# Kelicious/faster_rcnn

Measured on AMD Instinct MI355X. Metric: images/sec end-to-end (RPN+det) ResNet-50 600x1000, higher is better.
Workload: dtype f32

## Files before the change

faster_rcnn_amd/_lib.py:

```python
import ctypes
import os
from ctypes import c_char_p, c_double, c_int, c_size_t, c_void_p

HERE = os.path.dirname(os.path.abspath(__file__))
LIB_PATH = os.environ.get("FRCNN_LIB_PATH") or os.path.join(HERE, "libfrcnn_hip.so")


class FrcnnError(RuntimeError):
    pass


ABI_VERSION = 110
P = c_void_p
I = c_int
SIGNATURES = {
    "frcnn_last_error": (c_char_p, []),
    "frcnn_version": (I, []),
    "frcnn_device_count": (I, []),
    "frcnn_preprocess_u8": (I, [P, c_size_t, P, P, P]),
    "frcnn_resize_cubic_taps": (I, [I, I, P]),
    "frcnn_resize_cubic_u8": (I, [P, I, I, P, P, I, I, I, P, P]),
    "frcnn_anchors_image": (I, [I, I, P, I, I, P, P]),
    "frcnn_anchors_conv": (I, [I, I, P, I, P, P]),
    "frcnn_cross_ious_f32": (I, [P, I, P, I, P, P]),
# ... 109 lines not shown
    "frcnn_annotate_u8": (I, [P, I, I, P, P, P, P, I, P, P, I, I, P, P]),
    "frcnn_vgg_conv1_bf16_packed_elems": (I, []),
    "frcnn_pack_vgg_conv1_weights_bf16": (I, [P, P, P]),
    "frcnn_vgg_conv1_bf16_fwd": (I, [P, I, I, I, P, P, P, P]),
    "frcnn_pool2d_fwd_bf16": (I, [P, I, I, I, I, I, I, P, P]),
}

VGG_CANVAS_VERSION = 1
EXT_SIGNATURES = {
    "frcnn_vgg_canvas_version": (I, []),
    "frcnn_pool2d_fwd_extents": (I, [P, I, I, I, I, P, P, P]),
    "frcnn_pool2d_fwd_bf16_extents": (I, [P, I, I, I, I, P, P, P]),
    "frcnn_vgg_conv1_bf16_fwd_extents": (I, [P, I, I, I, P, P, P, P, P]),
}

ROI_RES_VERSION = 1
ROI_TAP_BYTES = 32
ROI_RES_SIGNATURES = {
    "frcnn_roi_res_version": (I, []),
    "frcnn_roi_tap_table": (I, [I, I, I, P, I, I, I, I, I, P, P]),
    "frcnn_conv2d_roi_res_available": (I, [P, I, I]),
    "frcnn_conv2d_fwd_h3_roi_res": (I, [P, P, P, P, P, P, P, P, P, P, P, P, ctypes.c_float, ctypes.c_float, P]),
}


POOL_EPILOGUE_VERSION = 1
POOL_EPILOGUE_SIGNATURES = {
    "frcnn_pool_epilogue_version": (I, []),
    "frcnn_conv2d_pool_available": (I, [P, I, I, I]),
    "frcnn_conv2d_fwd_h3_pool": (I, [P, P, P, P, P, P, P, P, P, P, I, P, P, P, P]),
}


class RoiRes(ctypes.Structure):
    _fields_ = [("map", c_void_p), ("taps", c_void_p), ("fill", c_void_p), ("map_rows", ctypes.c_int32), ("reserved", ctypes.c_int32)]


PNG_VERSION = 1
PNG_SIGNATURES = {
    "frcnn_png_version": (I, []),
    "frcnn_png_band_rows": (I, []),
    "frcnn_png_bound": (c_size_t, [I, I]),
    "frcnn_png_workspace_bytes": (c_size_t, [I, I]),
    "frcnn_png_encode_u8": (I, [P, I, I, I, P, c_size_t, P, P, P]),
}

PNG_HUFF_VERSION = 1
PNG_HUFF_SIGNATURES = {
    "frcnn_png_huff_version": (I, []),
    "frcnn_png_huff_band_rows": (I, []),
    "frcnn_png_huff_bound": (c_size_t, [I, I]),
    "frcnn_png_huff_workspace_bytes": (c_size_t, [I, I]),
    "frcnn_png_huff_encode_u8": (I, [P, I, I, I, P, c_size_t, P, P, P]),
}

JPEG_VERSION = 1
JPEG_SIGNATURES = {
    "frcnn_jpeg_version": (I, []),
    "frcnn_jpeg_restart_mcus": (I, []),
    "frcnn_jpeg_header_bytes": (c_size_t, []),
    "frcnn_jpeg_bound": (c_size_t, [I, I]),
    "frcnn_jpeg_workspace_bytes": (c_size_t, [I, I]),
    "frcnn_jpeg_encode_u8": (I, [P, I, I, I, I, P, c_size_t, P, P, P]),
}

JPEG_OPT_VERSION = 1
# ... 281 lines not shown
class ColsumJob(ctypes.Structure):
    _fields_ = [(k, c_void_p) for k in ("g", "scale", "out")] + [(k, ctypes.c_int32) for k in ("m", "cout", "g_is_bf16", "reserved")]


_lib = None


def load():
    global _lib
    if _lib is not None:
        return _lib
    if not os.path.exists(LIB_PATH):
        raise FrcnnError(
            f"{LIB_PATH} is missing: build it with `python -m faster_rcnn_amd.build` "
            "(hipcc --offload-arch=gfx950).  There is no CPU fallback.")
    import torch
    lib = ctypes.CDLL(LIB_PATH)
    for name, (res, args) in SIGNATURES.items():
        fn = getattr(lib, name)
        fn.restype = res
        fn.argtypes = args
    for name, (res, args) in EXT_SIGNATURES.items():
        fn = getattr(lib, name)
        fn.restype = res
        fn.argtypes = args
    for name, (res, args) in ROI_RES_SIGNATURES.items():
        fn = getattr(lib, name)
        fn.restype = res
        fn.argtypes = args
    for name, (res, args) in POOL_EPILOGUE_SIGNATURES.items():
        fn = getattr(lib, name)
        fn.restype = res
        fn.argtypes = args
    for name, (res, args) in PNG_SIGNATURES.items():
        fn = getattr(lib, name)
        fn.restype = res
        fn.argtypes = args
    for name, (res, args) in PNG_HUFF_SIGNATURES.items():
        fn = getattr(lib, name)
        fn.restype = res
        fn.argtypes = args
    for name, (res, args) in JPEG_SIGNATURES.items():
        fn = getattr(lib, name)
        fn.restype = res
        fn.argtypes = args
    for name, (res, args) in JPEG_OPT_SIGNATURES.items():
        fn = getattr(lib, name)
        fn.restype = res
        fn.argtypes = args
    for name, (res, args) in JPEG_DEC_SIGNATURES.items():
        fn = getattr(lib, name)
        fn.restype = res
        fn.argtypes = args
    for name, (res, args) in JPEG_DEC_BATCH_SIGNATURES.items():
        fn = getattr(lib, name)
        fn.restype = res
        fn.argtypes = args
    for name, (res, args) in PNG_DEC_SIGNATURES.items():
        fn = getattr(lib, name)
        fn.restype = res
        fn.argtypes = args
    for name, (res, args) in PNG_DEC_FULL_SIGNATURES.items():
        fn = getattr(lib, name)
        fn.restype = res
        fn.argtypes = args
    for name, (res, args) in JPEG_DEC_FULL_SIGNATURES.items():
# ... 144 lines not shown
```

faster_rcnn_amd/csrc/conv_igemm.hip:

```cpp
#include "conv_f32_common.h"
#include "conv_policy.h"
#include "../../include/ext/frcnn_hip_roi_res.h"
#include "../../include/ext/frcnn_hip_pool_epilogue.h"

namespace frcnn {

template <int TM, int TN, bool GENERIC_A>
__global__ void __launch_bounds__(256) k_conv_igemm_f32(const ConvArgs p) {
    constexpr int BM = 64 * TM, BN = 64 * TN;
    constexpr int PA = BM / 32, PB = BN / 32;
    extern __shared__ __attribute__((aligned(16))) float smem[];
    float* As = smem;
    float* Bs = smem + 2 * BM * LDS_STRIDE;

    const int tid = threadIdx.x, lane = tid & 63, wave = tid >> 6;
    const int wm = wave >> 1, wn = wave & 1;
    const int li = lane & 31, lh = lane >> 5;

    const int nwg = p.tiles_m * p.tiles_n;
    const int logical = xcd_remap(blockIdx.x, nwg);
    const int tile_n = logical / p.tiles_m, tile_m = logical - tile_n * p.tiles_m;
    const int m0 = tile_m * BM, n0 = tile_n * BN;

    const int lrow = tid >> 3, lcol = (tid & 7) * 4;
    int a_h[PA], a_w[PA];
    size_t a_img[PA];
#pragma unroll
    for (int i = 0; i < PA; ++i) {
        const int m = m0 + lrow + 32 * i;
        if (m < p.M) {
            const int wo = m % p.Wo, t = m / p.Wo, ho = t % p.Ho, img = t / p.Ho;
            a_h[i] = ho * p.stride - p.pad_top;
            a_w[i] = wo * p.stride - p.pad_left;
            a_img[i] = (size_t)img * p.H * p.W * p.Cin;
        } else {
            a_h[i] = -(1 << 28); a_w[i] = 0; a_img[i] = 0;
// ... 856 lines not shown
    a.img_stride = a.layout ? d->cin : d->h * d->w * d->cin;
    a.inv_S = (65536 + d->kw - 1) / d->kw;
    auto al16 = [](const void* q) { return (reinterpret_cast<uintptr_t>(q) & 15) == 0; };
    a.vec_epi = !conv_knobs().scalar_epilogue && (d->cout & 3) == 0 && (a.ldy & 3) == 0 && al16(y) && (size_t)M * a.ldy * 4 < 0x7fffffffull
             && (!residual || ((a.ldres & 3) == 0 && al16(residual) && (size_t)M * a.ldres * 4 < 0x7fffffffull))
             && (!mask || (al16(mask) && (size_t)M * d->cout * 4 < 0x7fffffffull)) && (!scale || al16(scale)) && (!shift || al16(shift));
    auto dual_vec_epi = [&](int bn) {
        return a.vec_epi && dual->n1 % bn == 0 && (a.ldy2 & 3) == 0 && al16(dual->y2) && (size_t)M * a.ldy2 * 4 < 0x7fffffffull;
    };
    auto use_workspace = [&]() { a.tickets = (unsigned*)workspace; a.slabs = (float*)((char*)workspace + SPLITK_TICKET_BYTES); };
    hipStream_t s = as_stream(stream);
    const bool generic = (d->cin % BK) != 0;
    if (engine != FRCNN_ENGINE_NATIVE) {
        const bool h3 = engine == FRCNN_ENGINE_H3;
        const SplitRule& r = split_rule(engine);
        int (*launch)(const ConvArgs&, int, hipStream_t) = h3 ? launch_conv_h3 : launch_conv_x6;
        if (generic || d->kh * d->kw > 32) return fail(FRCNN_E_UNSUPPORTED, "conv2d_fwd_%s: cin %% 32 == 0 and at most 32 taps", r.name);
        if ((size_t)r.planes * d->cout * a.Kpad * 2 >= 0x7fffffffull) return fail(FRCNN_E_UNSUPPORTED, "conv2d_fwd_%s: filter planes over 2 GiB", r.name);
        if (h3 && (reinterpret_cast<uintptr_t>(w_packed) & 15)) return fail(FRCNN_E_ARG, "conv2d_fwd_h3: 16-byte aligned filter planes required");
        const int cfg = split_config(r, d, dual ? dual->n1 : 0), bn = r.tile_width(cfg);
        if (a.res_map) {
            if (roi_res_available(d, engine, a.x_planes != nullptr) != 1 || dual || mask || residual || a.res_planes || workspace)
                return fail(FRCNN_E_UNSUPPORTED, "conv2d_fwd_h3_roi_res: not available for this launch (frcnn_conv2d_roi_res_available)");
            if (y && !a.vec_epi) return fail(FRCNN_E_ARG, "conv2d_fwd_h3_roi_res: 16-byte addressable output rows required");
            if ((long long)a.res_map_rows * d->cout * 4 >= 0x7fffffffLL || M * 32 >= 0x7fffffffLL) return fail(FRCNN_E_UNSUPPORTED, "conv2d_fwd_h3_roi_res: map or tap table over 2 GiB");
        }
        if (a.pool_rows) {
            if (pool_available(d, engine, a.x_planes != nullptr, a.pool_rows) != 1 || dual || mask || a.res_planes || a.res_map || a.y_planes || workspace || !y)
                return fail(FRCNN_E_UNSUPPORTED, "conv2d_fwd_h3_pool: not available for this launch (frcnn_conv2d_pool_available)");
            if (!a.vec_epi) return fail(FRCNN_E_ARG, "conv2d_fwd_h3_pool: 16-byte addressable output and residual rows required");
            a.pool_groups = 256 / a.pool_rows < 1024 / 128 ? 256 / a.pool_rows : 1024 / 128;
        }
        if (planes_io) {
            if ((cfg != 86 && cfg != 85 && cfg != 82) || dual || mask || (!a.vec_epi && y) || d->ldy > 0)
                return fail(FRCNN_E_UNSUPPORTED, "conv2d_fwd_h3_planes: needs the 256x128 tile (>= 256 output tiles of 128x128; frcnn_conv2d_h3_config 86 / 82), a dense single-layer launch without a mask");
            if ((d->cout & 3) || (d->cin & 7)) return fail(FRCNN_E_UNSUPPORTED, "conv2d_fwd_h3_planes: cin %% 8 == 0 and cout %% 4 == 0");
            if (a.res_planes && (residual || (y && !a.vec_epi))) return fail(FRCNN_E_ARG, "conv2d_fwd_h3_planes: residual planes exclude an f32 residual and need 16-byte addressable output rows");
            if ((size_t)M * d->cout * 4 >= 0x7fffffffull || (size_t)d->n * d->h * d->w * d->cin * 4 >= 0x7fffffffull)
                return fail(FRCNN_E_UNSUPPORTED, "conv2d_fwd_h3_planes: tensor planes over 2 GiB");
            if (!y) a.vec_epi = 1;
        } else if (workspace && !dual) {
            if (const size_t need = split_workspace_bytes(r, d)) {
                if (workspace_bytes < need) return fail(FRCNN_E_WORKSPACE, "conv2d_fwd_%s: workspace needs %zu bytes", r.name, need);
                a.splits = split_slices(r, d);
                use_workspace();
                a.group_m = 0;
                return launch(a, split_sk_code(r, d), s);
            }
        }
        if (dual) a.vec_epi = dual_vec_epi(bn);
        a.group_m = split_group_m(d, bn);
        return launch(a, cfg, s);
    }
    int cfg = choose_config(d);
    if (dual) {
        cfg = dual_config(cfg);
        a.vec_epi = dual_vec_epi(native_tile_width(cfg));
    }
    a.group_m = native_group_m(d, cfg);
    cfg = workspace_config(d, cfg, workspace != nullptr);
    if (a.layout && (generic || cfg < 11 || d->kh * d->kw > 32))
        return fail(FRCNN_E_UNSUPPORTED, "conv2d_fwd: position-major layout needs cin %% 32 == 0, a tensor under 2 GiB and at most 32 taps");
    if (d->cin == 3) {
        if (a.layout) return fail(FRCNN_E_UNSUPPORTED, "conv2d_fwd: position-major layout needs cin %% 32 == 0");
        if ((size_t)d->n * d->h * d->w * 12 >= 0x7fffffffull) return fail(FRCNN_E_UNSUPPORTED, "conv2d_fwd: 3-channel input over 2 GiB");
        return launch_conv_cin3(a, s, d->tile % 100 != 32);
    }
// ... 134 lines not shown

int frcnn_conv2d_fwd_x6(const frcnn_conv_desc* d, const float* x, const void* w_planes_bf16,
                        const float* scale, const float* shift, const float* residual, const float* mask, float* y,
                        void* workspace, size_t workspace_bytes, void* stream) {
    return conv_fwd_impl(d, x, reinterpret_cast<const float*>(w_planes_bf16), scale, shift, residual, mask, y, nullptr, workspace, workspace_bytes, stream, FRCNN_ENGINE_X6);
}

int frcnn_conv2d_fwd_dual_x6(const frcnn_conv_desc* d, const float* x, const void* w_planes_bf16, const float* scale, const float* shift,
                             float* y1, int n1, int act1, float* y2, int act2, void* stream) {
    if (!d || !y2 || n1 <= 0 || n1 >= d->cout) return fail(FRCNN_E_ARG, "conv2d_fwd_dual_x6: need 0 < n1 < cout and two outputs");
    if (d->ldy > 0 || d->ldres > 0) return fail(FRCNN_E_ARG, "conv2d_fwd_dual_x6: dense outputs only (ldy = ldres = 0)");
    const DualOut dual = {n1, act1, y2, act2};
    return conv_fwd_impl(d, x, reinterpret_cast<const float*>(w_planes_bf16), scale, shift, nullptr, nullptr, y1, &dual, nullptr, 0, stream, FRCNN_ENGINE_X6);
}

int frcnn_conv2d_fwd_h3(const frcnn_conv_desc* d, const float* x, const float* x_amax, const void* w_planes_f16,
                        const float* scale, const float* shift, const float* residual, const float* mask, float* y, float* y_amax,
                        void* workspace, size_t workspace_bytes, void* stream) {
    if (!x_amax) return fail(FRCNN_E_ARG, "conv2d_fwd_h3: the input's magnitude record is required (frcnn_amax_f32 makes one)");
    return conv_fwd_impl(d, x, reinterpret_cast<const float*>(w_planes_f16), scale, shift, residual, mask, y, nullptr, workspace, workspace_bytes, stream, FRCNN_ENGINE_H3,
                         amax_args(x_amax, y_amax));
}

int frcnn_conv2d_fwd_dual_h3(const frcnn_conv_desc* d, const float* x, const float* x_amax, const void* w_planes_f16, const float* scale, const float* shift,
                             float* y1, int n1, int act1, float* y1_amax, float* y2, int act2, float* y2_amax, void* stream) {
    if (!d || !y2 || n1 <= 0 || n1 >= d->cout) return fail(FRCNN_E_ARG, "conv2d_fwd_dual_h3: need 0 < n1 < cout and two outputs");
    if (d->ldy > 0 || d->ldres > 0) return fail(FRCNN_E_ARG, "conv2d_fwd_dual_h3: dense outputs only (ldy = ldres = 0)");
    if (!x_amax) return fail(FRCNN_E_ARG, "conv2d_fwd_dual_h3: the input's magnitude record is required");
    const DualOut dual = {n1, act1, y2, act2};
    return conv_fwd_impl(d, x, reinterpret_cast<const float*>(w_planes_f16), scale, shift, nullptr, nullptr, y1, &dual, nullptr, 0, stream, FRCNN_ENGINE_H3,
                         amax_args(x_amax, y1_amax, y2_amax));
}

int frcnn_conv2d_fwd_h3_planes(const frcnn_conv_desc* d, const float* x, const frcnn_h3_planes* x_planes, const float* x_amax, const void* w_planes_f16,
                               const float* scale, const float* shift, const float* residual, const float* residual_amax,
                               float* y, float* y_amax, const frcnn_h3_planes* y_planes, float bound_c, float bound_d, void* stream) {
    return frcnn_conv2d_fwd_h3_planes_res(d, x, x_planes, x_amax, w_planes_f16, scale, shift, residual, nullptr, residual_amax, y, y_amax, y_planes, bound_c, bound_d, stream);
}

int frcnn_conv2d_roi_res_available(const frcnn_conv_desc* d, int engine, int x_is_planes) {
    if (!d) return fail(FRCNN_E_ARG, "conv2d_roi_res_available: null descriptor");
    if (engine != FRCNN_ENGINE_NATIVE && engine != FRCNN_ENGINE_X6 && engine != FRCNN_ENGINE_H3) return fail(FRCNN_E_ARG, "conv2d_roi_res_available: unknown engine %d", engine);
    return roi_res_available(d, engine, x_is_planes != 0);
}

int frcnn_conv2d_fwd_h3_roi_res(const frcnn_conv_desc* d, const float* x, const frcnn_h3_planes* x_planes, const float* x_amax,
                                const void* w_planes_f16, const float* scale, const float* shift, const frcnn_roi_res* res,
                                const float* residual_amax, float* y, float* y_amax, const frcnn_h3_planes* y_planes,
                                float bound_c, float bound_d, void* stream) {
    return conv_h3_planes_impl(d, x, x_planes, x_amax, w_planes_f16, scale, shift, nullptr, nullptr, res, residual_amax, y, y_amax, y_planes, bound_c, bound_d, stream);
}

int frcnn_conv2d_fwd_h3_planes_res(const frcnn_conv_desc* d, const float* x, const frcnn_h3_planes* x_planes, const float* x_amax, const void* w_planes_f16,
                                   const float* scale, const float* shift, const float* residual, const frcnn_h3_planes* residual_planes,
                                   const float* residual_amax, float* y, float* y_amax, const frcnn_h3_planes* y_planes, float bound_c, float bound_d,
                                   void* stream) {
    return conv_h3_planes_impl(d, x, x_planes, x_amax, w_planes_f16, scale, shift, residual, residual_planes, nullptr, residual_amax, y, y_amax, y_planes, bound_c, bound_d, stream);
}

}

static int conv_h3_planes_impl(const frcnn_conv_desc* d, const float* x, const frcnn_h3_planes* x_planes, const float* x_amax, const void* w_planes_f16,
                               const float* scale, const float* shift, const float* residual, const frcnn_h3_planes* residual_planes,
                               const frcnn_roi_res* gathered, const float* residual_amax, float* y, float* y_amax, const frcnn_h3_planes* y_planes,
                               float bound_c, float bound_d, void* stream) {
    if (gathered) {
// ... 24 lines not shown
```

faster_rcnn_amd/nets.py:

```python
import os as _os

import numpy as np
import torch

from . import ops
from .weights import VGG_CONVS, resnet_block_names

BN_EPS_STEM = 1e-3
BN_EPS_BLOCK = 1e-5


class ConvUnit:

    def __init__(self, weights, conv, bn=None, scale=None, eps=BN_EPS_BLOCK, stride=1, padding="valid", act=None, tile=0,
                 dtype="f32", out_f32=False):
        self.weights, self.conv, self.bn, self.scale_name, self.eps = weights, conv, bn, scale, eps
        self.stride, self.padding, self.act, self.tile = stride, padding, act, tile
        self.dtype, self.out_f32 = dtype, out_f32
        self.pc = None

    def folded(self):
        w = self.weights[self.conv]
        kernel = np.asarray(w[0], dtype=np.float32)
        if kernel.ndim == 2:
# ... 33 lines not shown
        h, w = (x.shape[0], x.shape[1]) if layout else (x.shape[1], x.shape[2])
        return ops.conv2d_avgpool(x, self.pc, self.stride, self.padding, self.act, residual, h * w, self.tile, layout)


class DualUnit:

    def __init__(self, first, second):
        assert first.dtype == second.dtype == "f32" and (first.stride, first.padding) == (second.stride, second.padding)
        self.a, self.b, self.pc, self.n1 = first, second, None, None
        self._src = None

    def lower(self):
        a, b = self.a, self.b
        for u in (a, b):
            if u.pc is None:
                u.lower()
        wa, wb = a.pc.w, b.pc.w
        pc = ops.PackedConv.__new__(ops.PackedConv)
        pc.kh, pc.kw, pc.cin, pc.cout = a.pc.kh, a.pc.kw, a.pc.cin, a.pc.cout + b.pc.cout
        assert (a.pc.kh, a.pc.kw, a.pc.cin) == (b.pc.kh, b.pc.kw, b.pc.cin)
        pc.w = torch.cat([wa, wb], dim=0).contiguous()
        pc.scale = torch.cat([a.pc.scale, b.pc.scale]).contiguous()
        pc.shift = torch.cat([a.pc.shift, b.pc.shift]).contiguous()
        self.pc, self.n1, self._src = pc, a.pc.cout, (a.pc, b.pc)
        return self

    def __call__(self, x, act1="unit", act2="unit", layout=0):
        if self.pc is None or self._src[0] is not self.a.pc or self._src[1] is not self.b.pc:
            self.lower()
        act1 = self.a.act if act1 == "unit" else act1
        act2 = self.b.act if act2 == "unit" else act2
        return ops.conv2d_dual(x, self.pc, self.n1, self.a.stride, self.a.padding, act1, act2, layout, self.a.tile)


FUSE_PAIRS = True
FUSED_BF16_STEM = True
FUSED_F32_STEM = True


def _pair(first, second):
    if not FUSE_PAIRS or first.dtype != "f32" or second.dtype != "f32":
        return None
    d = getattr(first, "_dual", None)
    if d is None or d.b is not second:
        w = first.weights[first.conv][0]
        if np.ndim(w) != 4 or np.shape(w)[2] % 32 != 0:
            return None
        d = first._dual = DualUnit(first, second)
    return d


def _block_units(weights, stage, block, has_shortcut, stride, separate_scale, dtype="f32"):
    def unit(suffix, **kw):
        tag = "%d%s_branch%s" % (stage, block, suffix)
        return ConvUnit(weights, "res" + tag, "bn" + tag, ("scale" + tag) if separate_scale else None, BN_EPS_BLOCK, dtype=dtype, **kw)
    u = {"2a": unit("2a", stride=stride, act="relu"),
         "2b": unit("2b", padding="same", act="relu"),
         "2c": unit("2c", act="relu")}
    if has_shortcut:
        u["1"] = unit("1", stride=stride)
    return u


HEAD_PLANES = True
HEAD_BLOCK_PLANES = _os.environ.get("FRCNN_HEAD_BLOCK_PLANES", "0") != "0"
HEAD_ROI_RES = _os.environ.get("FRCNN_HEAD_ROI_RES", "1") != "0"
HEAD_POOL_EPI = _os.environ.get("FRCNN_HEAD_POOL_EPI", "1") != "0"
VGG_PLANES = _os.environ.get("FRCNN_VGG_PLANES", "1") != "0"
TRUNK_PLANES = _os.environ.get("FRCNN_TRUNK_PLANES", "0") != "0"


class Extents:
    LEVELS = 3
    CONV_LEVEL = 2

    @staticmethod
    def offset_of(height, width):
        return height & 1, width & 1

    def __init__(self, batch, pinned=None):
        self.batch = int(batch)
        n = self.LEVELS * self.batch * 2
        if pinned is not None:
            self.host = pinned[:4 * n].view(torch.int32).view(self.LEVELS, self.batch, 2)
            self.host.zero_()
        else:
            self.host = torch.zeros((self.LEVELS, self.batch, 2), dtype=torch.int32).pin_memory()
        self.table = torch.zeros((self.LEVELS, self.batch, 2), dtype=torch.int32, device="cuda")

    @staticmethod
    def levels_of(height, width):
        out = []
        h, w = (height - 1) // 2 + 1, (width - 1) // 2 + 1
        h, w = (h - 3) // 2 + 1, (w - 3) // 2 + 1
        out.append((h, w))
        for _ in range(2):
            h, w = (h - 1) // 2 + 1, (w - 1) // 2 + 1
            out.append((h, w))
        return out

    def set(self, i, height, width):
        for lvl, (h, w) in enumerate(self.levels_of(height, width)):
# ... 85 lines not shown
        for b in self.blocks:
            yield from b.values()

    def invalidate_fused(self, only=None):
        if only is None or self.stem.conv in only or self.stem.bn in only or self.stem.scale_name in only:
            self._stem_bf16 = None
            self._stem_h3 = None

    def lower_fused_stem(self):
        if self.dtype != "bf16" or not FUSED_BF16_STEM:
            return None
        src = tuple(id(a) for name in (self.stem.conv, self.stem.bn, self.stem.scale_name) if name for a in self.weights[name])
        if getattr(self, "_stem_bf16", None) is None or self._stem_src != src:
            self._stem_bf16, self._stem_src = ops.PackedStemBf16(*self.stem.folded()), src
        return self._stem_bf16

    def lower_fused_stem_h3(self):
        src = tuple(id(a) for name in (self.stem.conv, self.stem.bn, self.stem.scale_name) if name for a in self.weights[name])
        if getattr(self, "_stem_h3", None) is None or self._stem_h3_src != src:
            self._stem_h3, self._stem_h3_src = ops.PackedStemH3(*self.stem.folded()), src
        return self._stem_h3

    def stem_pool(self, x):
        if self.dtype == "bf16" and FUSED_BF16_STEM:
            return ops.stem_bf16(x, self.lower_fused_stem())
        if self.dtype == "f32" and FUSED_F32_STEM and ops.F32_ENGINE == "f16x3" and x.shape[1] >= 7 and x.shape[2] >= 7:
            return ops.stem_h3(x, self.lower_fused_stem_h3())
        x = ops.pool2d(self.stem(x), 3, 2, True)
        return ops.cast_bf16(x) if self.dtype == "bf16" else x

    def __call__(self, x, extents=None):
        x = self.stem_pool(x)
        planes = TRUNK_PLANES and self.dtype == "f32" and extents is None
        for b, lvl in zip(self.blocks, self.block_level):
            x = run_block(b, x, planes=planes, mask=None if extents is None else extents.level(lvl))
        if extents is not None:
            x = ops.zero_outside(x, extents.conv_map())
        return x


class VggBase:
    stride = 16
    out_channels = 512
    extents_class = VggExtents
    canvas_by_default = False

    def __init__(self, weights, dtype="f32"):
        assert dtype in ("f32", "bf16"), dtype
        self.weights, self.dtype = weights, dtype
        self.convs = [(name, ConvUnit(weights, name, padding="same", act="relu", dtype="f32" if name == "block1_conv1" else dtype))
                      for name, _, _ in VGG_CONVS]
        self._conv1_bf16 = None

    def units(self):
        for _, u in self.convs:
            yield u

    POOLED = ("block1_conv2", "block2_conv2", "block3_conv3", "block4_conv3")

    def invalidate_fused(self, only=None):
        if only is None or self.convs[0][0] in only:
            self._conv1_bf16 = None

    def lower_conv1_bf16(self):
        src = tuple(id(a) for a in self.weights[self.convs[0][0]])
        if self._conv1_bf16 is None or self._conv1_src != src:
            kernel, _, shift = self.convs[0][1].folded()
            self._conv1_bf16, self._conv1_src = ops.PackedVggConv1Bf16(kernel, shift), src
# ... 20 lines not shown
                x = pool(x, extents.level(lvl))
                lvl += 1
            else:
                x = ops.zero_outside(x, extents.level(lvl))
        return x

    def __call__(self, x, extents=None):
        if extents is not None:
            return self._forward_canvas(x, extents)
        if self.dtype == "bf16":
            return self._forward_bf16(x)
        for k, (name, u) in enumerate(self.convs):
            nxt = self.convs[k + 1][1] if (k + 1 < len(self.convs) and name not in self.POOLED) else None
            planes = VGG_PLANES and nxt is not None and _reads_planes(nxt, tuple(x.shape[:-1]) + (_cout(u),), 0)
            x = u(x, planes_out=planes)
            if name in self.POOLED:
                after = self.convs[k + 1][1] if k + 1 < len(self.convs) else None
                pooled = (x.shape[0], ops.valid_out(x.shape[1], 2, 2), ops.valid_out(x.shape[2], 2, 2), x.shape[3])
                x = ops.pool2d(x, 2, 2, True, planes_out=VGG_PLANES and after is not None and _reads_planes(after, pooled, 0))
        return x


class RpnHead:

    def __init__(self, weights, dtype="f32"):
        self.conv = ConvUnit(weights, "rpn_conv1", padding="same", act="relu", dtype=dtype)
        self.cls = ConvUnit(weights, "rpn_out_cls", act="sigmoid", dtype=dtype, out_f32=True)
        self.reg = ConvUnit(weights, "rpn_out_bbreg", dtype=dtype, out_f32=True)

    def units(self):
        return [self.conv, self.cls, self.reg]

    def __call__(self, feat):
        t = self.conv(feat)
        pair = _pair(self.cls, self.reg)
        if pair is not None and t.dtype == torch.float32:
            return pair(t)
        return self.cls(t), self.reg(t)


class _MergedDenseUnit(ConvUnit):

    def __init__(self, weights, num_classes):
        super().__init__(weights, "dense")
        self.names = ("dense_class_%d" % num_classes, "dense_reg_%d" % num_classes)

    def folded(self):
        (kc, bc), (kr, br) = (self.weights[n] for n in self.names)
        merged = {"dense": [np.concatenate([kc, kr], axis=1), np.concatenate([bc, br])]}
        return ConvUnit(merged, "dense").folded()


class _MergedDense:

    def __init__(self, weights, num_classes):
        self.C = num_classes
        self.unit = _MergedDenseUnit(weights, num_classes)

    def __call__(self, x2d):
        n, cin = x2d.shape
        y = self.unit(x2d.reshape(n, 1, 1, cin)).reshape(n, -1)
        return ops.dense_heads_split(y, self.C)


BATCHED_F32_HEAD_LAYOUT = int(_os.environ.get("FRCNN_BATCHED_HEAD_LAYOUT", "0"))
BATCHED_BF16_HEAD_LAYOUT = int(_os.environ.get("FRCNN_BATCHED_HEAD_LAYOUT_BF16", "1"))


class ResNetHead:
    pool = 7

    def __init__(self, weights, depth, num_classes, dtype="f32", hoist=True, pos_major=True):
        r101 = depth == 101
        self.dtype, self.hoist = dtype, hoist
        self.layout = 1 if (pos_major and _os.environ.get("FRCNN_HEAD_POS_MAJOR", "1") != "0") else 0
        self.blocks = [_block_units(weights, 5, b, b == "a", 1, r101, dtype) for b in "abc"]
        self.dense = _MergedDense(weights, num_classes)

    def units(self):
        for b in self.blocks:
            yield from b.values()
        yield self.dense.unit

    def _first_block_hoisted(self, feat, rois, resize, layout=None, n_per_img=0):
        a = self.blocks[0]
        if feat.dim() == 4 and feat.shape[0] > 1:
            fmap = feat
        else:
            fmap = ops.amax_carry(feat.reshape(1, feat.shape[-3], feat.shape[-2], feat.shape[-1]), feat)
        pair = _pair(a["2a"], a["1"])
        if pair is not None:
            u, v = pair(fmap, act1=None)
        else:
            u = a["2a"](fmap, act=None)
            v = a["1"](fmap)
        L = self.layout if layout is None else layout
        planes = self.dtype == "f32" and HEAD_PLANES
        n = rois.reshape(-1, 4).shape[0]
        crop_shape = (self.pool, self.pool, n, u.shape[-1]) if L else (n, self.pool, self.pool, u.shape[-1])
        if planes and _reads_planes(a["2b"], crop_shape, L):
            t = resize(u, rois, self.pool, fill=a["2a"].pc.shift, relu=True, layout=L, planes_out=True)
        else:
            t = resize(u, rois, self.pool, fill=a["2a"].pc.shift, relu=True, layout=L)
        out_shape = crop_shape[:-1] + (_cout(a["2c"]),)
        nxt = self.blocks[1] if len(self.blocks) > 1 else None
        t = a["2b"](t, layout=L, planes_out=planes and _reads_planes(a["2c"], crop_shape[:-1] + (_cout(a["2b"]),), L))
        c = a["2c"]
        if c.pc is None:
            c.lower()
        if HEAD_ROI_RES and self.dtype == "f32":
            s = ops.roi_shortcut(v, rois, self.pool, t, c.pc, fill=a["1"].pc.shift, layout=L, n_per_img=n_per_img,
                                 stride=c.stride, padding=c.padding, act=c.act, tile=c.tile)
        else:
            s = resize(v, rois, self.pool, fill=a["1"].pc.shift, layout=L)
        return c(t, residual=s, layout=L, planes_out=planes and nxt is not None and block_takes_planes(nxt, out_shape, L))

    def _run_rest(self, x, rest, L, pool=False):
        for i, b in enumerate(rest):
            nxt = rest[i + 1] if i + 1 < len(rest) else None
            x = run_block(b, x, L, planes=self.dtype == "f32", pool=pool and nxt is None,
                          out_planes=self.dtype == "f32" and nxt is not None and block_takes_planes(nxt, tuple(x.shape[:-1]) + (_cout(b["2c"]),), L))
        return x

    def __call__(self, feat, rois):
        resize = ops.roi_crop_resize_bf16 if self.dtype == "bf16" else ops.roi_crop_resize
        L = self.layout
        if self.hoist:
            x = self._first_block_hoisted(feat, rois, resize)
# ... 79 lines not shown
```

faster_rcnn_amd/ops.py:

```python
import ctypes
import dataclasses
import os

import numpy as np
import torch

from . import _lib
from . import y4m as _y4m

NMS_MAX_BOXES = 12288


_GPU_SEEN = False


def _require_gpu():
    global _GPU_SEEN
    if not _GPU_SEEN:
        if not torch.cuda.is_available():
            raise _lib.FrcnnError("no HIP device visible: the faster_rcnn_amd ops need an MI355X (no CPU fallback)")
        _GPU_SEEN = True


_RAW_STREAM = getattr(torch._C, "_cuda_getCurrentRawStream", None)
# ... 391 lines not shown
        self._h3_spread_log2 = _channel_spread_log2(w, 2)

    def x6_planes(self):
        planes = getattr(self, "_x6", None)
        if planes is None or getattr(self, "_x6_src", None) is not self.w:
            planes = torch.empty((3,) + tuple(self.w.shape), dtype=torch.bfloat16, device="cuda")
            _lib.call("frcnn_pack_conv_weights_x6", _p(self.w), self.w.shape[0], self.w.shape[1], _p(planes), _stream())
            self._x6, self._x6_src = planes, self.w
        return planes


    def h3_planes(self):
        planes = getattr(self, "_h3", None)
        if planes is None or getattr(self, "_h3_src", None) is not self.w:
            planes = torch.empty(_lib.load().frcnn_conv_h3_planes_bytes(self.w.shape[0], self.w.shape[1]), dtype=torch.uint8, device="cuda")
            _lib.call("frcnn_pack_conv_weights_h3", _p(self.w), self.w.shape[0], self.w.shape[1], _p(planes), _stream())
            self._h3, self._h3_src = planes, self.w
        return planes


    def h3_bound(self):
        b = getattr(self, "_h3_bound", None)
        if b is None or getattr(self, "_h3_bound_src", None) is not self.w:
            l1 = self.w.abs().sum(dim=1)
            if self.scale is not None:
                l1 = l1 * self.scale.abs()
            b = (float(l1.max().item()), 0.0 if self.shift is None else float(self.shift.abs().max().item()))
            self._h3_bound, self._h3_bound_src = b, self.w
        return b


class PlaneTensor:
    is_planes = True

    def __init__(self, shape):
        self.shape = tuple(int(v) for v in shape)
        self.planes = torch.empty((2,) + self.shape, dtype=torch.float16, device="cuda")
        self.exponent = torch.empty(1, dtype=torch.int32, device="cuda")
        self._amax = None

    def float(self):
        e = self.exponent.to(torch.float64)
        return ((self.planes[0].double() + self.planes[1].double() / 2048.0) * torch.pow(torch.tensor(2.0, dtype=torch.float64, device="cuda"), -e)).float()


F32_ENGINE = "native"
X6_MIN_TILES = 256
X6_MIN_COUT = 64


class f32_engine:
    def __init__(self, name):
        assert name in ("native", "bf16x6", "f16x3")
        self.name = name

    def __enter__(self):
        global F32_ENGINE
        self.prev, F32_ENGINE = F32_ENGINE, self.name

    def __exit__(self, *exc):
        global F32_ENGINE
        F32_ENGINE = self.prev


_ENGINE_CODE = {"native": 0, "bf16x6": 1, "f16x3": 2}
_ENGINE_TAG = {0: None, 1: "x6", 2: "h3"}
# ... 103 lines not shown
        stamp = getattr(rec, "_arena_gen", None)
        if stamp is not None and stamp[0].gen != stamp[1]:
            rec = None
            try:
                x._amax = None
            except AttributeError:
                pass
    if rec is None:
        global AMAX_MEASURED
        AMAX_MEASURED += 1
        rec = _amax_new()
        _lib.call("frcnn_amax_f32", _p(x), x.numel(), _p(rec), _stream())
    return rec


def amax_carry(dst, src, floor=0.0, exponent_out=None):
    rec = getattr(src, "_amax", None)
    stamp = getattr(rec, "_arena_gen", None) if rec is not None else None
    if stamp is not None and stamp[0].gen != stamp[1]:
        rec = None
    if rec is None:
        if exponent_out is not None:
            rec = amax_of(src)
        else:
            return dst
    if floor > 0.0 or exponent_out is not None:
        merged = _amax_new()
        _lib.call("frcnn_amax_merge", _p(merged), _p(rec), float(floor), _p(exponent_out), _stream())
        rec = merged
    dst._amax = rec
    return dst


def conv_accepts_planes(x_shape, pc, stride=1, padding="valid", act=None, layout=0, tile=0):
    if F32_ENGINE != "f16x3" or not isinstance(pc, PackedConv):
        return False
    d = _conv_desc(tuple(x_shape), pc.kh, pc.kw, pc.cout, stride, padding, ACT[act], layout, tile or AUTO_TILE)
    return _planes_ok(d, pc, _split_engine(d, pc, tile or AUTO_TILE))


H3_KERNEL_NAMES = {81: "k_conv_igemm_h3<2,1,2,4>", 82: "k_conv_igemm_h3_db<2,2,4,2>", 83: "k_conv_igemm_h3<2,2,2,2>", 84: "k_conv_igemm_h3<1,1,2,2>",
                   85: "k_conv_igemm_h3_db<2,1,4,4>", 86: "k_conv_igemm_h3_db<2,1,4,4>", 87: "k_conv_igemm_h3<2,1,2,2>"}


def _h3_name(d, n1=0):
    return H3_KERNEL_NAMES[_lib.load().frcnn_conv2d_h3_config(ctypes.byref(d), n1)]


X6_KERNEL_NAMES = {71: "k_conv_igemm_x6<2,1,2,4>", 72: "k_conv_igemm_x6<2,2,4,2>", 73: "k_conv_igemm_x6<2,2,2,2>", 74: "k_conv_igemm_x6<1,1,2,2>",
                   75: "k_conv_igemm_x6<1,1,2,4>", 76: "k_conv_igemm_x6_db", 77: "k_conv_igemm_x6<2,1,2,2>"}


def _x6_name(d, n1=0):
    return X6_KERNEL_NAMES[_lib.load().frcnn_conv2d_x6_config(ctypes.byref(d), n1)]


CONV_PROFILE = None
CONV_KERNEL_NAMES = {1: "k_conv_igemm_f32<2,2,false>", 2: "k_conv_igemm_f32<1,1,*>", 3: "k_conv_igemm_f32<2,1,*>",
                     4: "k_conv_igemm_f32<4,2,false>", 11: "k_conv_igemm_f32_v2<2,2>", 12: "k_conv_igemm_f32_v2<1,1>",
                     13: "k_conv_igemm_f32_v2<2,1>", 14: "k_conv_igemm_f32_v2<4,2>",
                     21: "k_conv_igemm_f32_v2<2,2,1>", 22: "k_conv_igemm_f32_v2<1,1,1>",
                     23: "k_conv_igemm_f32_v2<1,1,2>", 24: "k_conv_igemm_f32_v2<1,2,2>", 25: "k_conv_igemm_f32_v2<2,1,2>", 26: "k_conv_igemm_f32_v2<2,2,2>",
                     30: "k_conv_igemm_f32_v2<1,1,2> stem", 32: "k_conv_igemm_f32_v2<1,1,1> stem", 61: "k_conv_igemm_f32_sk<2,2>", 62: "k_conv_igemm_f32_sk<1,1>", 41: "k_conv_igemm_f32_v2<1,2,1,4,2>", 42: "k_conv_igemm_f32_v2<2,1,1,2,4>", 43: "k_conv_igemm_f32_v2<1,1,1,4,2>"}


def _record_launch(kernel, shape, fn, args, keep, **extra):
    if CONV_PROFILE is None:
        return
    CONV_PROFILE.append({"kernel": kernel(), **extra, "flops": 2.0 * shape[0] * shape[1] * shape[2], "shape": shape,
                         "relaunch": lambda fn=fn, args=args, keep=keep: _lib.call(fn, *args, _stream())})

# ... 57 lines not shown
        self.ws = ws

    def __enter__(self):
        global _CONV_WS
        self.prev, _CONV_WS = _CONV_WS, self.ws
        return self.ws

    def __exit__(self, *exc):
        global _CONV_WS
        _CONV_WS = self.prev


def _split_k_ws(need):
    if not need or _CONV_WS is NO_SPLIT_K:
        return None
    holder = _CONV_WS
    if holder is None and not torch.cuda.is_current_stream_capturing():
        holder = _STREAM_WS.setdefault(torch.cuda.current_stream().cuda_stream, ConvWorkspace())
    return None if holder is None else holder.get(need)


def _conv_launch(d, x, w, scale, shift, residual, mask, out, y_amax=None):
    ws = _split_k_ws(_ws_need(d, "frcnn_conv2d_workspace_bytes"))
    head = (ctypes.byref(d), _p(x), _p(w), _p(scale), _p(shift), _p(residual), _p(mask), _p(out))
    tail = (_p(ws), ws.numel() if ws is not None else 0)
    fn, args = ("frcnn_conv2d_fwd_ws", head + tail) if y_amax is None else ("frcnn_conv2d_fwd_ws_amax", head + (_p(y_amax),) + tail)
    _lib.call(fn, *args, _stream())
    return (fn, args), ws


def _conv2d_h3_planes(d, x, pc, residual, oshape, planes_out, act):
    x_in = isinstance(x, PlaneTensor)
    xp = _lib.H3Planes(planes=x.planes.data_ptr(), exponent=x.exponent.data_ptr(), status=None) if x_in else None
    y = PlaneTensor(oshape) if planes_out else torch.empty(oshape, dtype=torch.float32, device="cuda")
    ya = _amax_new()
    yp = _lib.H3Planes(planes=y.planes.data_ptr(), exponent=y.exponent.data_ptr(), status=ya.data_ptr() + 4) if planes_out else None
    bc, bd = pc.h3_bound() if planes_out else (0.0, 0.0)
    xa = amax_of(x)
    r_in = isinstance(residual, PlaneTensor)
    r_roi = isinstance(residual, RoiResidual)
    ra = (residual.amax() if r_roi else amax_of(residual)) if (residual is not None and planes_out) else None
    rp = _lib.H3Planes(planes=residual.planes.data_ptr(), exponent=residual.exponent.data_ptr(), status=None) if r_in else None
    head = (ctypes.byref(d), None if x_in else _p(x), ctypes.byref(xp) if x_in else None, _p(xa), _p(pc.h3_planes()), _p(pc.scale), _p(pc.shift))
    tail = (_p(ra), None if planes_out else _p(y), _p(ya), ctypes.byref(yp) if planes_out else None, bc, bd)
    if r_roi:
        rp = residual.desc()
        fn, args = "frcnn_conv2d_fwd_h3_roi_res", head + (ctypes.byref(rp),) + tail
    else:
        fn, args = "frcnn_conv2d_fwd_h3_planes_res", head + (None if r_in else _p(residual), ctypes.byref(rp) if r_in else None) + tail
    _lib.call(fn, *args, _stream())
    y._amax = ya
    _record_launch(lambda: _h3_planes_in_name(d, pc) if x_in else _h3_name(d), _gemm_shape(d, pc, d.stride), fn,
                   args, (d, x, pc, residual, y, ya, xp, yp, xa, ra, rp), planes_out=bool(planes_out), roi_res=bool(r_roi))
    return y


def _h3_planes_in_name(d, pc):
    return _h3_name(d).replace(">", ",planes>")


def _planes_ok(d, pc, eng):
    return (eng == "h3" and _lib.load().frcnn_conv2d_h3_config(ctypes.byref(d), 0) in (86, 85, 82) and pc.cout % 4 == 0 and pc.cin % 8 == 0
            and (_CONV_WS is NO_SPLIT_K or _ws_need(d, "frcnn_conv2d_h3_workspace_bytes") == 0))


def conv2d(x, pc, stride=1, padding="valid", act=None, residual=None, out=None, tile=0, layout=0, planes_out=False):
    _require_gpu()
    x_planes = isinstance(x, PlaneTensor)
    assert (x_planes or (x.dtype == torch.float32 and x.is_contiguous())) and x.shape[-1] == pc.cin, (x.shape, pc.cin)
    d = _conv_desc(tuple(x.shape), pc.kh, pc.kw, pc.cout, stride, padding, ACT[act], layout, tile or AUTO_TILE)
    n, ho, wo = d.n, d.ho, d.wo
    oshape = (ho, wo, n, pc.cout) if layout else (n, ho, wo, pc.cout)
    res_planes = isinstance(residual, PlaneTensor)
    roi_res = isinstance(residual, RoiResidual)
    if x_planes or planes_out or res_planes or roi_res:
        ok = out is None and _planes_ok(d, pc, _split_engine(d, pc, tile or AUTO_TILE))
        if roi_res and not (ok and conv_takes_roi_res(x, pc, stride, padding, act, layout, tile)):
            raise _lib.FrcnnError("conv2d: this launch cannot gather a RoiResidual (ops.conv_takes_roi_res; frcnn_conv2d_roi_res_available)")
        if (x_planes or res_planes) and not ok:
            raise _lib.FrcnnError("conv2d: a PlaneTensor input / residual needs an f16x3 launch on the 256x128 tile (frcnn_conv2d_fwd_h3_planes)")
        if ok:
            if residual is not None:
                assert tuple(residual.shape) == tuple(oshape) and (res_planes or roi_res or residual.is_contiguous())
            return _conv2d_h3_planes(d, x, pc, residual, oshape, planes_out, act)
    if out is None:
        out = torch.empty(oshape, dtype=torch.float32, device="cuda")
    else:
        assert out.shape == oshape and out.is_contiguous()
    if residual is not None:
        assert residual.shape == out.shape and residual.is_contiguous()
    eng = _split_engine(d, pc, tile or AUTO_TILE)
    ya = xa = None
    if eng is None:
        ya = _amax_new(optional=True) if (_tracking() and pc.cout >= 32) else None
        (fn, args), ws = _conv_launch(d, x, pc.w, pc.scale, pc.shift, residual, None, out, ya)
    else:
        fn = "frcnn_conv2d_fwd_" + eng
        ws = _split_k_ws(_ws_need(d, f"frcnn_conv2d_{eng}_workspace_bytes"))
        tail = (_p(pc.scale), _p(pc.shift), _p(residual), None, _p(out))
        if eng == "h3":
            ya, xa = _amax_new(), amax_of(x)
            args = (ctypes.byref(d), _p(x), _p(xa), _p(pc.h3_planes())) + tail + (_p(ya),)
        else:
            args = (ctypes.byref(d), _p(x), _p(pc.x6_planes())) + tail
        args += (_p(ws), ws.numel() if ws is not None else 0)
        _lib.call(fn, *args, _stream())
    if ya is not None or getattr(out, "_amax", None) is not None:
        out._amax = ya
    _record_launch(lambda: _kernel_name(d, eng, ws), _gemm_shape(d, pc, stride), fn, args, (d, x, pc, residual, out, ws, ya, xa))
    return out


def conv2d_dual(x, pc, n1, stride=1, padding="valid", act1=None, act2=None, layout=0, tile=0):
    _require_gpu()
    assert x.dtype == torch.float32 and x.is_contiguous() and x.shape[-1] == pc.cin and 0 < n1 < pc.cout
    d = _conv_desc(tuple(x.shape), pc.kh, pc.kw, pc.cout, stride, padding, 0, layout, tile or AUTO_TILE)
    lead = (d.ho, d.wo, d.n) if layout else (d.n, d.ho, d.wo)
    y1 = torch.empty(lead + (n1,), dtype=torch.float32, device="cuda")
    y2 = torch.empty(lead + (pc.cout - n1,), dtype=torch.float32, device="cuda")
    eng = _split_engine(d, pc, tile or AUTO_TILE)
    ws = a1 = a2 = xa = None
    outs = (_p(y1), n1, ACT[act1], _p(y2), ACT[act2])
    if eng == "h3":
        a1, a2, xa = _amax_new(), _amax_new(), amax_of(x)
        args = (ctypes.byref(d), _p(x), _p(xa), _p(pc.h3_planes()), _p(pc.scale), _p(pc.shift), _p(y1), n1, ACT[act1], _p(a1),
                _p(y2), ACT[act2], _p(a2))
    elif eng == "x6":
        args = (ctypes.byref(d), _p(x), _p(pc.x6_planes()), _p(pc.scale), _p(pc.shift)) + outs
    else:
        ws = _split_k_ws(_ws_need(d, "frcnn_conv2d_dual_workspace_bytes"))
        args = (ctypes.byref(d), _p(x), _p(pc.w), _p(pc.scale), _p(pc.shift)) + outs + (_p(ws), ws.numel() if ws is not None else 0)
    fn = "frcnn_conv2d_fwd_dual" + (f"_{eng}" if eng else "")
    _lib.call(fn, *args, _stream())
    if eng == "h3":
        y1._amax, y2._amax = a1, a2
    _record_launch(lambda: _kernel_name(d, eng, ws, n1), _gemm_shape(d, pc, stride), fn, args, (d, x, pc, y1, y2, ws, a1, a2, xa))
    return y1, y2


def pool2d(x, k, stride, is_max=True, planes_out=False):
    _require_gpu()
    n, h, w, c = x.shape
    ho, wo = valid_out(h, k, stride), valid_out(w, k, stride)
    if planes_out and F32_ENGINE == "f16x3" and _tracking() and c % 4 == 0:
        out = PlaneTensor((n, ho, wo, c))
        amax_carry(out, x, 0.0, exponent_out=out.exponent)
        yp = _lib.H3Planes(planes=out.planes.data_ptr(), exponent=out.exponent.data_ptr(), status=out._amax.data_ptr() + 4)
        _lib.call("frcnn_pool2d_fwd_planes", _p(x.contiguous()), n, h, w, c, k, stride, 1 if is_max else 0, ctypes.byref(yp), _stream())
        return out
    out = torch.empty((n, ho, wo, c), dtype=torch.float32, device="cuda")
    _lib.call("frcnn_pool2d_fwd", _p(x.contiguous()), n, h, w, c, k, stride, 1 if is_max else 0, _p(out), _stream())
    return amax_carry(out, x)


def conv_takes_pool(x, pc, stride=1, padding="valid", act=None, layout=0, tile=0, window=49):
# ... 1662 lines not shown
```

Baseline: 566.8.

## Emit conv4 trunk output as both f32 and f16x3 planes for RPN/head reuse

The last trunk block now writes its output both as a dense f32 tensor and as pre-split f16x3 planes. The RPN conv and the detection head's first paired/dual convolutions then read those planes directly instead of re-splitting the f32 feature map. A new dual-output plane-input entry point and a relaxed planes_io check make the paired 1x1/2a conv able to take plane input. This costs an extra plane write per image and more memory, and adds staleness checks so the planes twin is only reused when its arena generation still matches.

```diff
diff --git a/faster_rcnn_amd/_lib.py b/faster_rcnn_amd/_lib.py
--- a/faster_rcnn_amd/_lib.py
+++ b/faster_rcnn_amd/_lib.py
@@ -165,6 +165,13 @@
 }
 
 
+CONV4_PLANES_VERSION = 1
+CONV4_PLANES_SIGNATURES = {
+    "frcnn_conv4_planes_version": (I, []),
+    "frcnn_conv2d_fwd_dual_h3_planes": (I, [P, P, P, P, P, P, P, I, I, P, P, I, P, P]),
+}
+
+
 class RoiRes(ctypes.Structure):
     _fields_ = [("map", c_void_p), ("taps", c_void_p), ("fill", c_void_p), ("map_rows", ctypes.c_int32), ("reserved", ctypes.c_int32)]
 
@@ -512,6 +519,15 @@
         fn = getattr(lib, name)
         fn.restype = res
         fn.argtypes = args
+    for name, (res, args) in CONV4_PLANES_SIGNATURES.items():
+        fn = getattr(lib, name, None)
+        if fn is None:
+            raise FrcnnError(f"{LIB_PATH} has no {name} (include/ext/frcnn_hip_conv4_planes.h): rebuild with `python -m faster_rcnn_amd.build`")
+        fn.restype = res
+        fn.argtypes = args
+    if lib.frcnn_conv4_planes_version() != CONV4_PLANES_VERSION:
+        raise FrcnnError(f"{LIB_PATH} speaks revision {lib.frcnn_conv4_planes_version()} of the paired plane-input extension, this binding "
+                         f"{CONV4_PLANES_VERSION} (include/ext/frcnn_hip_conv4_planes.h): rebuild with `python -m faster_rcnn_amd.build`")
     for name, (res, args) in PNG_SIGNATURES.items():
         fn = getattr(lib, name)
         fn.restype = res
diff --git a/faster_rcnn_amd/csrc/conv_igemm.hip b/faster_rcnn_amd/csrc/conv_igemm.hip
--- a/faster_rcnn_amd/csrc/conv_igemm.hip
+++ b/faster_rcnn_amd/csrc/conv_igemm.hip
@@ -2,6 +2,7 @@
 #include "conv_policy.h"
 #include "../../include/ext/frcnn_hip_roi_res.h"
 #include "../../include/ext/frcnn_hip_pool_epilogue.h"
+#include "../../include/ext/frcnn_hip_conv4_planes.h"
 
 namespace frcnn {
 
@@ -924,7 +925,7 @@
             a.pool_groups = 256 / a.pool_rows < 1024 / 128 ? 256 / a.pool_rows : 1024 / 128;
         }
         if (planes_io) {
-            if ((cfg != 86 && cfg != 85 && cfg != 82) || dual || mask || (!a.vec_epi && y) || d->ldy > 0)
+            if ((cfg != 86 && cfg != 85 && cfg != 82) || (dual && (a.y_planes || a.res_planes || residual || !dual_vec_epi(bn))) || mask || (!a.vec_epi && y) || d->ldy > 0)
                 return fail(FRCNN_E_UNSUPPORTED, "conv2d_fwd_h3_planes: needs the 256x128 tile (>= 256 output tiles of 128x128; frcnn_conv2d_h3_config 86 / 82), a dense single-layer launch without a mask");
             if ((d->cout & 3) || (d->cin & 7)) return fail(FRCNN_E_UNSUPPORTED, "conv2d_fwd_h3_planes: cin %% 8 == 0 and cout %% 4 == 0");
             if (a.res_planes && (residual || (y && !a.vec_epi))) return fail(FRCNN_E_ARG, "conv2d_fwd_h3_planes: residual planes exclude an f32 residual and need 16-byte addressable output rows");
@@ -1125,6 +1126,22 @@
                          amax_args(x_amax, y1_amax, y2_amax));
 }
 
+int frcnn_conv4_planes_version(void) { return FRCNN_CONV4_PLANES_VERSION; }
+
+int frcnn_conv2d_fwd_dual_h3_planes(const frcnn_conv_desc* d, const frcnn_h3_planes* x_planes, const float* x_amax, const void* w_planes_f16,
+                                    const float* scale, const float* shift, float* y1, int n1, int act1, float* y1_amax,
+                                    float* y2, int act2, float* y2_amax, void* stream) {
+    if (!d || !y1 || !y2 || n1 <= 0 || n1 >= d->cout) return fail(FRCNN_E_ARG, "conv2d_fwd_dual_h3_planes: need 0 < n1 < cout and two outputs");
+    if (d->ldy > 0 || d->ldres > 0) return fail(FRCNN_E_ARG, "conv2d_fwd_dual_h3_planes: dense outputs only (ldy = ldres = 0)");
+    if (!x_amax) return fail(FRCNN_E_ARG, "conv2d_fwd_dual_h3_planes: the input's magnitude record is required");
+    if (!x_planes || !x_planes->planes || !x_planes->exponent || (reinterpret_cast<uintptr_t>(x_planes->planes) & 15))
+        return fail(FRCNN_E_ARG, "conv2d_fwd_dual_h3_planes: incomplete or misaligned input planes");
+    const DualOut dual = {n1, act1, y2, act2};
+    ConvArgs rg = amax_args(x_amax, y1_amax, y2_amax);
+    rg.x_planes = x_planes->planes; rg.x_pexp = x_planes->exponent;
+    return conv_fwd_impl(d, nullptr, reinterpret_cast<const float*>(w_planes_f16), scale, shift, nullptr, nullptr, y1, &dual, nullptr, 0, stream, FRCNN_ENGINE_H3, rg);
+}
+
 int frcnn_conv2d_fwd_h3_planes(const frcnn_conv_desc* d, const float* x, const frcnn_h3_planes* x_planes, const float* x_amax, const void* w_planes_f16,
                                const float* scale, const float* shift, const float* residual, const float* residual_amax,
                                float* y, float* y_amax, const frcnn_h3_planes* y_planes, float bound_c, float bound_d, void* stream) {
diff --git a/faster_rcnn_amd/nets.py b/faster_rcnn_amd/nets.py
--- a/faster_rcnn_amd/nets.py
+++ b/faster_rcnn_amd/nets.py
@@ -89,6 +89,11 @@
         act2 = self.b.act if act2 == "unit" else act2
         return ops.conv2d_dual(x, self.pc, self.n1, self.a.stride, self.a.padding, act1, act2, layout, self.a.tile)
 
+    def reads_planes(self, x_shape, layout=0):
+        if self.pc is None or self._src[0] is not self.a.pc or self._src[1] is not self.b.pc:
+            self.lower()
+        return ops.conv_accepts_planes(tuple(x_shape), self.pc, self.a.stride, self.a.padding, None, layout, self.a.tile, n1=self.n1)
+
 
 FUSE_PAIRS = True
 FUSED_BF16_STEM = True
@@ -125,6 +130,7 @@
 HEAD_POOL_EPI = _os.environ.get("FRCNN_HEAD_POOL_EPI", "1") != "0"
 VGG_PLANES = _os.environ.get("FRCNN_VGG_PLANES", "1") != "0"
 TRUNK_PLANES = _os.environ.get("FRCNN_TRUNK_PLANES", "0") != "0"
+CONV4_PLANES = _os.environ.get("FRCNN_CONV4_PLANES", "1") != "0"
 
 
 class Extents:
@@ -276,8 +282,10 @@
     def __call__(self, x, extents=None):
         x = self.stem_pool(x)
         planes = TRUNK_PLANES and self.dtype == "f32" and extents is None
+        twin = CONV4_PLANES and self.dtype == "f32" and extents is None
         for b, lvl in zip(self.blocks, self.block_level):
-            x = run_block(b, x, planes=planes, mask=None if extents is None else extents.level(lvl))
+            x = run_block(b, x, planes=planes, mask=None if extents is None else extents.level(lvl),
+                          out_planes="both" if (twin and b is self.blocks[-1]) else False)
         if extents is not None:
             x = ops.zero_outside(x, extents.conv_map())
         return x
@@ -364,7 +372,11 @@
         return [self.conv, self.cls, self.reg]
 
     def __call__(self, feat):
-        t = self.conv(feat)
+        twin = ops.planes_twin(feat) if (CONV4_PLANES and self.conv.dtype == "f32") else None
+        if twin is not None and _reads_planes(self.conv, feat.shape, 0):
+            t = self.conv(twin)
+        else:
+            t = self.conv(feat)
         pair = _pair(self.cls, self.reg)
         if pair is not None and t.dtype == torch.float32:
             return pair(t)
@@ -421,11 +433,14 @@
         else:
             fmap = ops.amax_carry(feat.reshape(1, feat.shape[-3], feat.shape[-2], feat.shape[-1]), feat)
         pair = _pair(a["2a"], a["1"])
+        twin = ops.planes_twin(feat) if (CONV4_PLANES and self.dtype == "f32") else None
+        if twin is not None and tuple(twin.shape) != tuple(fmap.shape):
+            twin = None
         if pair is not None:
-            u, v = pair(fmap, act1=None)
-        else:
-            u = a["2a"](fmap, act=None)
-            v = a["1"](fmap)
+            u, v = pair(twin if (twin is not None and pair.reads_planes(fmap.shape)) else fmap, act1=None)
+        else:
+            u = a["2a"](twin if (twin is not None and _reads_planes(a["2a"], fmap.shape, 0)) else fmap, act=None)
+            v = a["1"](twin if (twin is not None and _reads_planes(a["1"], fmap.shape, 0)) else fmap)
         L = self.layout if layout is None else layout
         planes = self.dtype == "f32" and HEAD_PLANES
         n = rois.reshape(-1, 4).shape[0]
diff --git a/faster_rcnn_amd/ops.py b/faster_rcnn_amd/ops.py
--- a/faster_rcnn_amd/ops.py
+++ b/faster_rcnn_amd/ops.py
@@ -447,6 +447,7 @@
 
 class PlaneTensor:
     is_planes = True
+    twin = False
 
     def __init__(self, shape):
         self.shape = tuple(int(v) for v in shape)
@@ -616,11 +617,11 @@
     return dst
 
 
-def conv_accepts_planes(x_shape, pc, stride=1, padding="valid", act=None, layout=0, tile=0):
+def conv_accepts_planes(x_shape, pc, stride=1, padding="valid", act=None, layout=0, tile=0, n1=0):
     if F32_ENGINE != "f16x3" or not isinstance(pc, PackedConv):
         return False
-    d = _conv_desc(tuple(x_shape), pc.kh, pc.kw, pc.cout, stride, padding, ACT[act], layout, tile or AUTO_TILE)
-    return _planes_ok(d, pc, _split_engine(d, pc, tile or AUTO_TILE))
+    d = _conv_desc(tuple(x_shape), pc.kh, pc.kw, pc.cout, stride, padding, 0 if n1 else ACT[act], layout, tile or AUTO_TILE)
+    return _planes_ok(d, pc, _split_engine(d, pc, tile or AUTO_TILE), n1)
 
 
 H3_KERNEL_NAMES = {81: "k_conv_igemm_h3<2,1,2,4>", 82: "k_conv_igemm_h3_db<2,2,4,2>", 83: "k_conv_igemm_h3<2,2,2,2>", 84: "k_conv_igemm_h3<1,1,2,2>",
@@ -744,9 +745,11 @@
 def _conv2d_h3_planes(d, x, pc, residual, oshape, planes_out, act):
     x_in = isinstance(x, PlaneTensor)
     xp = _lib.H3Planes(planes=x.planes.data_ptr(), exponent=x.exponent.data_ptr(), status=None) if x_in else None
-    y = PlaneTensor(oshape) if planes_out else torch.empty(oshape, dtype=torch.float32, device="cuda")
+    both = planes_out == "both"
+    yt = PlaneTensor(oshape) if planes_out else None
+    y = torch.empty(oshape, dtype=torch.float32, device="cuda") if (both or not planes_out) else yt
     ya = _amax_new()
-    yp = _lib.H3Planes(planes=y.planes.data_ptr(), exponent=y.exponent.data_ptr(), status=ya.data_ptr() + 4) if planes_out else None
+    yp = _lib.H3Planes(planes=yt.planes.data_ptr(), exponent=yt.exponent.data_ptr(), status=ya.data_ptr() + 4) if planes_out else None
     bc, bd = pc.h3_bound() if planes_out else (0.0, 0.0)
     xa = amax_of(x)
     r_in = isinstance(residual, PlaneTensor)
@@ -754,7 +757,7 @@
     ra = (residual.amax() if r_roi else amax_of(residual)) if (residual is not None and planes_out) else None
     rp = _lib.H3Planes(planes=residual.planes.data_ptr(), exponent=residual.exponent.data_ptr(), status=None) if r_in else None
     head = (ctypes.byref(d), None if x_in else _p(x), ctypes.byref(xp) if x_in else None, _p(xa), _p(pc.h3_planes()), _p(pc.scale), _p(pc.shift))
-    tail = (_p(ra), None if planes_out else _p(y), _p(ya), ctypes.byref(yp) if planes_out else None, bc, bd)
+    tail = (_p(ra), _p(y) if (both or not planes_out) else None, _p(ya), ctypes.byref(yp) if planes_out else None, bc, bd)
     if r_roi:
         rp = residual.desc()
         fn, args = "frcnn_conv2d_fwd_h3_roi_res", head + (ctypes.byref(rp),) + tail
@@ -762,18 +765,36 @@
         fn, args = "frcnn_conv2d_fwd_h3_planes_res", head + (None if r_in else _p(residual), ctypes.byref(rp) if r_in else None) + tail
     _lib.call(fn, *args, _stream())
     y._amax = ya
-    _record_launch(lambda: _h3_planes_in_name(d, pc) if x_in else _h3_name(d), _gemm_shape(d, pc, d.stride), fn,
-                   args, (d, x, pc, residual, y, ya, xp, yp, xa, ra, rp), planes_out=bool(planes_out), roi_res=bool(r_roi))
+    if both:
+        yt._amax, yt.twin = ya, True
+        y._planes = yt
+    _record_launch(lambda: _h3_planes_in_name(d, pc, x) if x_in else _h3_name(d), _gemm_shape(d, pc, d.stride) + (("both",) if both else ()), fn,
+                   args, (d, x, pc, residual, y, yt, ya, xp, yp, xa, ra, rp), planes_out=bool(planes_out), roi_res=bool(r_roi))
     return y
 
 
-def _h3_planes_in_name(d, pc):
-    return _h3_name(d).replace(">", ",planes>")
-
-
-def _planes_ok(d, pc, eng):
-    return (eng == "h3" and _lib.load().frcnn_conv2d_h3_config(ctypes.byref(d), 0) in (86, 85, 82) and pc.cout % 4 == 0 and pc.cin % 8 == 0
-            and (_CONV_WS is NO_SPLIT_K or _ws_need(d, "frcnn_conv2d_h3_workspace_bytes") == 0))
+def planes_twin(x):
+    t = getattr(x, "_planes", None)
+    rec = getattr(x, "_amax", None)
+    if t is None or rec is None or t._amax is not rec or tuple(t.shape) != tuple(x.shape):
+        return None
+    stamp = getattr(rec, "_arena_gen", None)
+    if stamp is not None and stamp[0].gen != stamp[1]:
+        return None
+    return t
+
+
+def _h3_planes_in_name(d, pc, x=None, n1=0):
+    name = _h3_name(d, n1).replace(">", ",planes>")
+    return name + " twin" if getattr(x, "twin", False) else name
+
+
+def _planes_ok(d, pc, eng, n1=0):
+    if not (eng == "h3" and _lib.load().frcnn_conv2d_h3_config(ctypes.byref(d), n1) in (86, 85, 82) and pc.cout % 4 == 0 and pc.cin % 8 == 0):
+        return False
+    if n1:
+        return n1 % 128 == 0 and (pc.cout - n1) % 4 == 0
+    return _CONV_WS is NO_SPLIT_K or _ws_need(d, "frcnn_conv2d_h3_workspace_bytes") == 0
 
 
 def conv2d(x, pc, stride=1, padding="valid", act=None, residual=None, out=None, tile=0, layout=0, planes_out=False):
@@ -825,7 +846,8 @@
 
 def conv2d_dual(x, pc, n1, stride=1, padding="valid", act1=None, act2=None, layout=0, tile=0):
     _require_gpu()
-    assert x.dtype == torch.float32 and x.is_contiguous() and x.shape[-1] == pc.cin and 0 < n1 < pc.cout
+    x_planes = isinstance(x, PlaneTensor)
+    assert (x_planes or (x.dtype == torch.float32 and x.is_contiguous())) and x.shape[-1] == pc.cin and 0 < n1 < pc.cout
     d = _conv_desc(tuple(x.shape), pc.kh, pc.kw, pc.cout, stride, padding, 0, layout, tile or AUTO_TILE)
     lead = (d.ho, d.wo, d.n) if layout else (d.n, d.ho, d.wo)
     y1 = torch.empty(lead + (n1,), dtype=torch.float32, device="cuda")
@@ -833,6 +855,18 @@
     eng = _split_engine(d, pc, tile or AUTO_TILE)
     ws = a1 = a2 = xa = None
     outs = (_p(y1), n1, ACT[act1], _p(y2), ACT[act2])
+    if x_planes:
+        if not _planes_ok(d, pc, eng, n1):
+            raise _lib.FrcnnError("conv2d_dual: a PlaneTensor input needs an f16x3 launch on the 256x128 tile (frcnn_conv2d_fwd_dual_h3_planes)")
+        a1, a2, xa = _amax_new(), _amax_new(), amax_of(x)
+        xp = _lib.H3Planes(planes=x.planes.data_ptr(), exponent=x.exponent.data_ptr(), status=None)
+        fn = "frcnn_conv2d_fwd_dual_h3_planes"
+        args = (ctypes.byref(d), ctypes.byref(xp), _p(xa), _p(pc.h3_planes()), _p(pc.scale), _p(pc.shift), _p(y1), n1, ACT[act1], _p(a1),
+                _p(y2), ACT[act2], _p(a2))
+        _lib.call(fn, *args, _stream())
+        y1._amax, y2._amax = a1, a2
+        _record_launch(lambda: _h3_planes_in_name(d, pc, x, n1), _gemm_shape(d, pc, stride), fn, args, (d, x, pc, y1, y2, a1, a2, xa, xp))
+        return y1, y2
     if eng == "h3":
         a1, a2, xa = _amax_new(), _amax_new(), amax_of(x)
         args = (ctypes.byref(d), _p(x), _p(xa), _p(pc.h3_planes()), _p(pc.scale), _p(pc.shift), _p(y1), n1, ACT[act1], _p(a1),
diff --git a/include/ext/frcnn_hip_conv4_planes.h b/include/ext/frcnn_hip_conv4_planes.h
--- /dev/null
+++ b/include/ext/frcnn_hip_conv4_planes.h
@@ -0,0 +1,19 @@
+#ifndef FRCNN_HIP_CONV4_PLANES_H
+#define FRCNN_HIP_CONV4_PLANES_H
+#include <stdint.h>
+#include "../frcnn_hip.h"
+#ifdef __cplusplus
+extern "C" {
+#endif
+
+#define FRCNN_CONV4_PLANES_VERSION 1
+int frcnn_conv4_planes_version(void);
+
+int frcnn_conv2d_fwd_dual_h3_planes(const frcnn_conv_desc* d, const frcnn_h3_planes* x_planes, const float* x_amax, const void* w_planes_f16,
+                                    const float* scale, const float* shift, float* y1, int n1, int act1, float* y1_amax,
+                                    float* y2, int act2, float* y2_amax, void* stream);
+
+#ifdef __cplusplus
+}
+#endif
+#endif
```

New measurement: 571.8, median of 6. About the same (+0.9%).
